# nullstyle/capnp-zig

Hardware: AMD Instinct MI355X
Metric: GiB/s device-resident packed encode+decode, 1M x 4KiB segments (higher is better)
Workload: dtype u8; 1 GPU; 1048576 units x 4096 B per GPU, zero-byte p=128/256, encode into capacity slots + decode from slots; units_per_gpu=1048576, unit_bytes=4096, zero_thresh=128, parallelism=shard1

## Files before the change

### capnp-zig_amd/csrc/packed_kernels.hip

```cpp
#include <hip/hip_runtime.h>
#include <stdint.h>
#include <stdio.h>
#include <stdlib.h>

#include <algorithm>
#include <atomic>
#include <map>
#include <memory>
#include <mutex>
#include <string>
#include <type_traits>
#include <vector>

#include "capnp_packed.h"
#include "class_ws.h"
#include "kernels.h"

namespace cpk {

constexpr int kWave = 64;
constexpr int kWavesPerBlock = 4;
constexpr int kBlock = kWave * kWavesPerBlock;

constexpr uint32_t kEncMaxWords = 512;
// ... 2808 lines not shown
                m_T = (uint32_t)(out_len[uu] >> 3);
                m_st = status[uu];
            }
        }
    };
    auto meta = [&](uint32_t j) {
        FillMeta m;
        m.st = (int32_t)readlane((uint32_t)m_st, j);
        m.P = readlane(m_P, j);
        m.src = in + ((uint64_t)readlane((uint32_t)m_in, j) | ((uint64_t)readlane((uint32_t)(m_in >> 32), j) << 32));
        m.dst = out + ((uint64_t)readlane((uint32_t)m_out, j) | ((uint64_t)readlane((uint32_t)(m_out >> 32), j) << 32));
        m.T = readlane(m_T, j);
        m.rec = reinterpret_cast<const uint16_t*>((uint64_t)readlane((uint32_t)m_rec, j) |
                                                  ((uint64_t)readlane((uint32_t)(m_rec >> 32), j) << 32));
        return m;
    };

    uint4 v0, v1, v2, v3, v4;
    uint32_t r0 = 0, r1 = 0, r2 = 0, r3 = 0, r4 = 0;
    auto load_unit = [&](const FillMeta& m) {
        const bool go = m.st == ST_OK && m.P > 0;
        if (!go) return;
        const uint32_t s = (uint32_t)(reinterpret_cast<uintptr_t>(m.src) & 15);
        const uint4* const b = reinterpret_cast<const uint4*>(m.src - s);
        const uint32_t np = (s + m.P + 15) >> 4;
        const uint32_t last = np - 1;
        v0 = load_nt(b + min(lane, last));
        if (np > 64) v1 = load_nt(b + min(lane + 64, last));
        if (np > 128) v2 = load_nt(b + min(lane + 128, last));
        if (np > 192) v3 = load_nt(b + min(lane + 192, last));
        if (np > 256) v4 = load_nt(b + min(lane + 256, last));
        const uint32_t L = (np + 63) >> 6;
        const uint16_t* const rc = m.rec;
        const uint32_t q = lane * L + 1;
        r0 = rc[min(q, np)];
        if (L > 1) r1 = rc[min(q + 1, np)];
        if (L > 2) r2 = rc[min(q + 2, np)];
        if (L > 3) r3 = rc[min(q + 3, np)];
        if (L > 4) r4 = rc[min(q + 4, np)];
    };

    load_batch(0);
    FillMeta cur = meta(0);
    load_unit(cur);
    uint32_t younger = 0;
    for (uint32_t k = 0; (uint64_t)u0 + (uint64_t)k * G < n; ++k) {
        const bool go = cur.st == ST_OK && cur.P > 0;
        vmcnt_at_most(younger);
        younger = 0;
        uint32_t np = 0, end = 0, pos = 0, words = 0, jend = 0;
        if (go) {
            const uint32_t s = (uint32_t)(reinterpret_cast<uintptr_t>(cur.src) & 15);
            end = s + cur.P;
            np = (end + 15) >> 4;
            wave_lds_sync();
            uint4* const pk4 = reinterpret_cast<uint4*>(pk);
            pk4[lane] = v0;
            if (np > 64) pk4[lane + 64] = v1;
            if (np > 128) pk4[lane + 128] = v2;
            if (np > 192) pk4[lane + 192] = v3;
            if (np > 256) pk4[lane + 256] = v4;
            const uint32_t L = (np + 63) >> 6;
            const uint32_t q0 = min(lane * L, np), q1 = min(q0 + L, np);
            const uint32_t nq = q1 - q0;
            jend = min(16 * q1, end);
            pos = jend;
            const uint32_t rr[kFlMaxL] = {r0, r1, r2, r3, r4};
#pragma unroll
            for (int i = kFlMaxL - 1; i >= 0; --i) {
                const uint32_t r = rr[i];
                const bool has = (uint32_t)i < nq && (r >> 4) != 0;
                words += has ? (r >> 4) : 0u;
                pos = has ? 16 * (q0 + i) + (r & 15u) : pos;
            }
        }
        const uint32_t k1 = k + 1;
        if ((k1 & 63) == 0) {
            asm volatile("s_waitcnt vmcnt(0)" ::: "memory");
            load_batch(k1);
        }
        const FillMeta nxt = meta(k1 & 63);
        load_unit(nxt);
        if (go) {
            const uint32_t incl = wave_incl_sum(words);
            const uint32_t wbase = incl - words;
            const bool a16 = !(reinterpret_cast<uintptr_t>(cur.dst) & 15);
            uint64_t* const dst = reinterpret_cast<uint64_t*>(cur.dst);
            const uint32_t T = cur.T;
            for (uint32_t W0 = 0; W0 < T; W0 += kFlOut) {
                const uint32_t W1 = min(T, W0 + kFlOut);
                wave_lds_sync();
                reinterpret_cast<uint4*>(code)[lane] = make_uint4(kFlZero * 0x10001u, kFlZero * 0x10001u,
                                                                  kFlZero * 0x10001u, kFlZero * 0x10001u);
                wave_lds_sync();
                const bool mine = words > 0 && wbase < W1 && wbase + words > W0;
                uint32_t p = mine ? pos : jend, w = wbase;
                bool runs = false;
                for (;;) {
                    const bool act = p < jend && w < W1;
                    if (__builtin_amdgcn_ballot_w64(act) == 0) break;
                    const uint32_t pp = act ? p : 0u;
                    uint32_t t = pk[pp];
                    uint32_t b1 = pk[pp + 1];
                    uint32_t c9 = pk[pp + 9];
                    asm volatile("" : "+v"(t), "+v"(b1), "+v"(c9));
                    const bool z = t == 0u, f = t == 0xFFu;
                    code[(act && !z && w >= W0) ? w - W0 : kFlOut] = (uint16_t)pp;
                    const uint32_t c = f ? c9 : 0u;
                    runs |= act && c != 0u;
                    if (act && c && w < W0) {
                        for (uint32_t i = W0 - w; i <= c && w + i < W1; ++i)
                            code[w + i - W0] = (uint16_t)(kFlLit | (pp + 1 + 8 * i));
                    }
                    w = act ? w + 1u + (z ? b1 : 0u) + c : w;
                    p = act ? p + 1u + __popc(t) + (uint32_t)(z | f) + 8u * c : p;
                }
                wave_lds_sync();
                if (__builtin_amdgcn_ballot_w64(runs) != 0) {
                    fl_bodies(pk, code, W1 - W0, lane);
                    wave_lds_sync();
                }
                const uint32_t nw = W1 - W0;
                if (a16) {
                    for (uint32_t i = 2 * lane; i < nw; i += 2 * kWave) {
                        const uint32_t cc = *reinterpret_cast<const uint32_t*>(code + i);
                        const uint64_t x0 = fill_word(pk, lut, cc & 0xFFFFu);
                        const uint64_t x1 = fill_word(pk, lut, cc >> 16);
                        if (i + 1 < nw) {
                            const u32x4 v = {(uint32_t)x0, (uint32_t)(x0 >> 32), (uint32_t)x1, (uint32_t)(x1 >> 32)};
                            __builtin_nontemporal_store(v, reinterpret_cast<u32x4*>(dst + W0 + i));
                        }
                        else dst[W0 + i] = x0;
                    }
                    younger += (nw + 2 * kWave - 1) / (2 * kWave);
                } else {
                    for (uint32_t i = lane; i < nw; i += kWave) dst[W0 + i] = fill_word(pk, lut, code[i]);
                    younger += (nw + kWave - 1) / kWave;
                }
            }
        }
        cur = nxt;
    }
    asm volatile("s_waitcnt vmcnt(0)" ::: "memory");
}

constexpr uint32_t kLwWaves = 2;
constexpr uint32_t kLwCarry = 12;
constexpr uint32_t kLwRing = kLwCarry + 64;
constexpr uint32_t kLwS = 8;
constexpr uint32_t kLwLine = 16;
constexpr uint32_t kLwLB = 8 * kLwLine;
constexpr uint32_t kLwLanes = kLwLB / 16;
constexpr uint32_t kLwLds = kLwWaves * kWave * (kLwRing + kLwLB + 2) + 128;
static_assert(kLwLds <= 26624, "six blocks per CU");

template <bool RD>
__global__ __launch_bounds__(kLwWaves * kWave) void decode_words_kernel(
    const uint8_t* __restrict__ in, const uint64_t* __restrict__ in_off, const uint64_t* __restrict__ in_len,
    uint32_t n, uint8_t* __restrict__ out, const uint64_t* __restrict__ out_off,
    const uint64_t* __restrict__ out_cap, uint64_t* __restrict__ out_len, int32_t* __restrict__ status,
    const uint32_t* __restrict__ list, const uint32_t* __restrict__ list_count,
    const uint32_t* __restrict__ list_lo, uint32_t* __restrict__ bail_count, uint64_t* __restrict__ consumed) {
    __shared__ __attribute__((aligned(16))) uint8_t ring_blk[kLwWaves * kWave * kLwRing];
    __shared__ __attribute__((aligned(16))) uint8_t line_blk[kLwWaves * kWave * kLwLB];
    __shared__ uint16_t ftab_blk[kLwWaves * kWave];
    __shared__ uint64_t nib[16];
    if (threadIdx.x < 16) {
        const uint64_t e = expand_selector(threadIdx.x);
        uint32_t m = 0;
        for (uint32_t k = 0; k < 4; ++k) m |= ((threadIdx.x >> k) & 1u) ? 0xFFu << (8 * k) : 0u;
        nib[threadIdx.x] = (e & 0xFFFFFFFFull) | ((uint64_t)m << 32);
    }
    __syncthreads();
    const uint32_t lane = lane_id();
    const uint32_t wave = threadIdx.x >> 6;
    uint8_t* const ring_all = ring_blk + wave * (kWave * kLwRing);
    uint8_t* const lines = line_blk + wave * (kWave * kLwLB);
    uint8_t* const myline = lines + lane * kLwLB;
    uint16_t* const ftab = ftab_blk + wave * kWave;
    const uint32_t wv = blockIdx.x * kLwWaves + wave;
    const uint32_t lo = list_lo ? *list_lo : 0u;
    const uint32_t count = (list ? *list_count : n) - lo;
    if (wv * kWave >= count) return;
    const uint32_t slot = wv * kWave + lane;
    const bool valid = slot < count;
    const uint32_t unit = valid ? ((list && (lo != 0 || count != n)) ? list[lo + slot] : slot) : 0u;

    const uint8_t* src = cpk_dummy16;
    uint64_t P64 = 0, cap = 0;
    uint8_t* dstb = nullptr;
    int32_t st = ST_OK;
    bool gated = false;
    uint64_t fw = 0;
    uint32_t past = 0;
    if (valid) {
        if (RD) gated = status[unit] != kStWords;
        src = in + in_off[unit];
        P64 = in_len[unit];
        dstb = out + out_off[unit];
        cap = out_cap[unit];
        if (RD) {
            fw = out_len[unit] >> 3;
            if (P64 > 10 * fw) {
                past = P64 - 10 * fw > (1u << 20) ? (1u << 20) : (uint32_t)(P64 - 10 * fw);
                P64 = 10 * fw;
            }
        }
        if (P64 > 0 && (reinterpret_cast<uintptr_t>(dstb) & 7)) st = ST_ARG;
        if (P64 >= kIxSizeMax) st = kStNeedFull;
    }
    const uint32_t s = (uint32_t)(reinterpret_cast<uintptr_t>(src) & 15);
    const bool take = valid && !gated && st == ST_OK && P64 > 0;
    const uint32_t end = take ? s + (uint32_t)P64 : 0u;
    const uint32_t npieces = (end + 15) >> 4;
    uint32_t maxr = (end + 63) >> 6;
#pragma unroll
    for (int d = 32; d >= 1; d >>= 1) maxr = max(maxr, (uint32_t)__shfl_xor((int)maxr, d, kWave));
    maxr = __builtin_amdgcn_readfirstlane(maxr);
    const uint32_t capw = (uint32_t)min(cap >> 3, (uint64_t)0x7FFFFFFFu);
    const uint32_t lim_w = RD ? (uint32_t)min(fw, (uint64_t)0x7FFFFFFFu) : capw;
    const uint32_t s0 = take ? (uint32_t)((reinterpret_cast<uintptr_t>(dstb) >> 3) & (kLwLine - 1)) : 0u;
    const uint64_t line0 = reinterpret_cast<uint64_t>(dstb) - 8ull * s0;

    const uint4* qsrc[4];
    uint32_t qlast[4];
#pragma unroll
    for (uint32_t m = 0; m < 4; ++m) {
        const uint32_t r = 16 * m + lane / 4;
        const uint64_t rb = __shfl(reinterpret_cast<uint64_t>(src - s), r, kWave);
        const uint32_t rn = __shfl(npieces, r, kWave);
        qsrc[m] = reinterpret_cast<const uint4*>(rn ? reinterpret_cast<const uint8_t*>(rb) : cpk_dummy16);
        qlast[m] = rn ? rn - 1 : 0u;
    }
    const uint32_t qp = lane & 3;
    u32x4 d0, d1, d2, d3;
    auto load = [&](uint32_t k) {
        ds_gload16(d0, qsrc[0] + min(4 * k + qp, qlast[0]));
        ds_gload16(d1, qsrc[1] + min(4 * k + qp, qlast[1]));
        ds_gload16(d2, qsrc[2] + min(4 * k + qp, qlast[2]));
        ds_gload16(d3, qsrc[3] + min(4 * k + qp, qlast[3]));
    };
    uint8_t* const wq = ring_all + (lane / 4) * kLwRing + kLwCarry + 16 * qp;
    auto put16 = [&](uint8_t* p, const u32x4& v) {
        uint32_t* const d = reinterpret_cast<uint32_t*>(p);
        d[0] = v.x;
        d[1] = v.y;
        d[2] = v.z;
        d[3] = v.w;
    };
    uint8_t* const ring = ring_all + lane * kLwRing;

    uint32_t younger = 0;
    auto flush = [&](bool want, uint64_t A, uint32_t lo, uint32_t hi) {
        const uint64_t F = __builtin_amdgcn_ballot_w64(want);
        if (F == 0) return;
        const uint32_t cnt = (uint32_t)__popcll(F);
        const uint32_t rk = __builtin_amdgcn_mbcnt_hi((uint32_t)(F >> 32), __builtin_amdgcn_mbcnt_lo((uint32_t)F, 0u));
        wave_lds_sync();
        if (want) ftab[rk] = (uint16_t)(lane | (lo << 6) | (hi << 10));
        wave_lds_sync();
        const uint32_t Alo = (uint32_t)A, Ahi = (uint32_t)(A >> 32);
        const uint32_t j = lane & (kLwLanes - 1);
        auto store16 = [&](uint32_t ent, uint64_t a, const u32x4& v, bool in_r) {
            const uint32_t flo = (ent >> 6) & 15u, fhi = ent >> 10;
            uint8_t* const p = reinterpret_cast<uint8_t*>(a) + 16 * j;
            if (__builtin_amdgcn_ballot_w64(in_r && (flo | (fhi ^ kLwLine)) != 0u) == 0) {
                ++younger;
                if (in_r) asm volatile("global_store_dwordx4 %0, %1, off nt\n\ts_nop 1" ::"v"(p), "v"(v));
                return;
            }
            const bool a0 = in_r && 2 * j >= flo && 2 * j < fhi, a1 = in_r && 2 * j + 1 >= flo && 2 * j + 1 < fhi;
            const bool both = a0 && a1, first = a0 && !a1, second = a1 && !a0;
            if (__builtin_amdgcn_ballot_w64(both) != 0) {
                ++younger;
                if (both) asm volatile("global_store_dwordx4 %0, %1, off nt\n\ts_nop 1" ::"v"(p), "v"(v));
            }
            if (__builtin_amdgcn_ballot_w64(first | second) != 0) {
                ++younger;
                uint8_t* const q = second ? p + 8 : p;
                const uint64_t x = second ? ((uint64_t)v.z | ((uint64_t)v.w << 32)) : ((uint64_t)v.x | ((uint64_t)v.y << 32));
                if (first | second) asm volatile("global_store_dwordx2 %0, %1, off nt\n\ts_nop 1" ::"v"(q), "v"(x));
            }
        };
        constexpr uint32_t kGrp = kWave / kLwLanes;
        for (uint32_t g = 0; g < cnt; g += 2 * kGrp) {
            const uint32_t ra = g + lane / kLwLanes, rb = ra + kGrp;
            const uint32_t ea = ftab[min(ra, cnt - 1)], eb = ftab[min(rb, cnt - 1)];
            const uint32_t ua = ea & 63u, ub = eb & 63u;
            const uint64_t aa = (uint64_t)(uint32_t)__shfl((int)Alo, (int)ua, kWave) |
                                ((uint64_t)(uint32_t)__shfl((int)Ahi, (int)ua, kWave) << 32);
            const uint64_t ab = (uint64_t)(uint32_t)__shfl((int)Alo, (int)ub, kWave) |
                                ((uint64_t)(uint32_t)__shfl((int)Ahi, (int)ub, kWave) << 32);
            const u32x4 va = *reinterpret_cast<const u32x4*>(lines + ua * kLwLB + 16 * j);
            const u32x4 vb = *reinterpret_cast<const u32x4*>(lines + ub * kLwLB + 16 * j);
            store16(ea, aa, va, ra < cnt);
            if (g + kGrp < cnt) store16(eb, ab, vb, rb < cnt);
        }
    };
    auto line_hi_cap = [&](uint32_t L, uint32_t hi) {
        const int64_t c = (int64_t)capw + s0 - (int64_t)kLwLine * L;
        return (uint32_t)max<int64_t>(0, min<int64_t>(hi, c));
    };

    constexpr int32_t kFar = 0x3FFFFFFF;
    int32_t po = take ? (int32_t)(s + kLwCarry) : kFar;
    int32_t end_o = take ? (int32_t)(end + kLwCarry) : 0;
    uint32_t run = 0, rsel = 0;
    int32_t apos = po;
    uint32_t W = 0;
    if (maxr > 0) load(0);
    uint32_t ksh = 0;
    for (uint32_t k = 0; k <= maxr; ++k) {
        if (__builtin_amdgcn_ballot_w64(take && W < lim_w && (po < end_o || run != 0u)) == 0) break;
        if (k < maxr) {
            vmcnt_at_most63(younger);
            asm volatile("" : "+v"(d0), "+v"(d1), "+v"(d2), "+v"(d3));
        }
        younger = 0;
        if (k > 0) {
            wave_lds_sync();
            uint32_t* const rd = reinterpret_cast<uint32_t*>(ring);
            const uint32_t c0 = rd[16], c1 = rd[17], c2 = rd[18];
            rd[0] = c0;
            rd[1] = c1;
            rd[2] = c2;
            wave_lds_sync();
            po -= 64;
            end_o -= 64;
            ++ksh;
            apos = apos == INT32_MIN ? apos : po;
        }
        if (k < maxr) {
            put16(wq, d0);
            put16(wq + 16 * kLwRing, d1);
            put16(wq + 32 * kLwRing, d2);
            put16(wq + 48 * kLwRing, d3);
            if (k + 1 < maxr) load(k + 1);
            wave_lds_sync();
        }
        const int32_t lim = min(64, end_o);
        const int32_t slim = min(67, end_o);
        for (;;) {
            if (__builtin_amdgcn_ballot_w64(run >= kLwLine && rsel == 0u) != 0) {
                const uint32_t wcap = min(lim_w, capw);
                const bool bz = rsel == 0u && run >= kLwLine && ((s0 + W) & (kLwLine - 1)) == 0u &&
                                W + kLwLine <= wcap;
                if (__builtin_amdgcn_ballot_w64(bz) != 0) {
                    const uint32_t nl = bz ? min(run, wcap - W) / kLwLine : 0u;
                    const uint32_t nmax = wave_max_u32(nl);
                    const u32x4 z = {0u, 0u, 0u, 0u};
                    for (uint32_t i = 0; i < nmax; ++i) {
                        if (i < nl) {
                            uint8_t* const zl = reinterpret_cast<uint8_t*>(line0 + (uint64_t)kLwLB * ((s0 + W) / kLwLine + i));
#pragma unroll
                            for (uint32_t c = 0; c < kLwLB / 16; ++c)
                                asm volatile("global_store_dwordx4 %0, %1, off nt\n\ts_nop 1" ::"v"(zl + 16 * c), "v"(z));
                        }
                        younger += kLwLB / 16;
                    }
                    W += kLwLine * nl;
                    run -= kLwLine * nl;
                    apos = (run != 0u && rsel == 0u) ? INT32_MIN : po;
                }
            }
            uint32_t rec[kLwS];
#pragma unroll
            for (uint32_t j = 0; j < kLwS; ++j) rec[j] = 0u;
            uint32_t e = 0;
            __builtin_amdgcn_s_setprio(1);
            const uint32_t rem = W < lim_w ? lim_w - W : 0u;
            const int32_t limx = rem != 0u ? slim : INT32_MIN;
#pragma unroll
            for (uint32_t j = 0; j < kLwS; ++j) {
                const bool act = apos < limx && (!RD || j < rem);
                if (__builtin_amdgcn_ballot_w64(act) == 0) break;
                if (act) {
                    const uint32_t o = (uint32_t)min(max(po, 0), 66);
                    const uint8_t* const a = ring + o;
                    uint32_t t = a[0], b1 = a[1], c9 = a[9];
                    asm volatile("" : "+v"(t), "+v"(b1), "+v"(c9));
                    const bool inrec = run == 0u;
                    const bool tz = t == 0u, tf = t == 0xFFu;
                    const uint32_t len = (uint32_t)__popc(t) + 1u + (uint32_t)(tz | tf);
                    const uint32_t cnt = tz ? b1 : (tf ? c9 : 0u);
                    const uint32_t tsel = inrec ? t : rsel;
                    rec[j] = (o + (uint32_t)inrec) | (tsel << 8);
                    po += (int32_t)(inrec ? len : (rsel & 8u));
                    run = inrec ? cnt : run - 1u;
                    rsel = inrec ? (tf ? 0xFFu : 0u) : rsel;
                    apos = (run != 0u && rsel == 0u) ? INT32_MIN : po;
                    e = j + 1;
                }
            }
            __builtin_amdgcn_s_setprio(0);
            uint64_t w[kLwS];
#pragma unroll
            for (uint32_t j = 0; j < kLwS; ++j) {
                const uint32_t r16 = rec[j];
                const uint32_t o = r16 & 0xFFu, sh = o & 3u;
                const uint32_t* const rw = reinterpret_cast<const uint32_t*>(ring + (o & ~3u));
                const uint32_t D0 = rw[0], D1 = rw[1], D2 = rw[2];
                const uint64_t pay = (uint64_t)__builtin_amdgcn_alignbyte(D1, D0, sh) |
                                     ((uint64_t)__builtin_amdgcn_alignbyte(D2, D1, sh) << 32);
                const uint32_t tg = r16 >> 8;
                const uint64_t elo = nib[tg & 15u], ehi = nib[tg >> 4];
                const uint32_t shi = (uint32_t)ehi + (((uint32_t)__popc(tg & 15u) * 0x01010101u) & (uint32_t)(ehi >> 32));
                w[j] = perm64(pay, (uint64_t)(uint32_t)elo | ((uint64_t)shi << 32));
            }
            const uint32_t sl = (s0 + W) & (kLwLine - 1);
            const uint32_t f = kLwLine - sl;
#pragma unroll
            for (uint32_t j = 0; j < kLwS; ++j)
                if (j < e && j < f) *reinterpret_cast<uint64_t*>(myline + 8 * ((sl + j) & (kLwLine - 1))) = w[j];
            const bool full = e >= f && e != 0u;
            if (__builtin_amdgcn_ballot_w64(full) != 0) {
                __builtin_amdgcn_s_setprio(1);
                const uint32_t L = (s0 + W) / kLwLine;
                flush(full, line0 + (uint64_t)kLwLB * L, L == 0 ? s0 : 0u, line_hi_cap(L, kLwLine));
                __builtin_amdgcn_s_setprio(0);
                wave_lds_sync();
#pragma unroll
                for (uint32_t j = 0; j < kLwS; ++j)
                    if (j < e && j >= f) *reinterpret_cast<uint64_t*>(myline + 8 * ((sl + j) & (kLwLine - 1))) = w[j];
            }
            W += e;
            if (__builtin_amdgcn_ballot_w64(apos < lim && W < lim_w) == 0) break;
        }
    }
    {
        const uint32_t L = (s0 + W) / kLwLine, hi = (s0 + W) & (kLwLine - 1);
        const bool part = take && hi != 0u;
        flush(part, line0 + (uint64_t)kLwLB * L, L == 0 ? s0 : 0u, line_hi_cap(L, hi));
    }
    asm volatile("s_waitcnt vmcnt(0)" ::: "memory");
    if (!valid || gated) return;
    if (st == kStNeedFull) {
        status[unit] = st;
        return;
    }
    if (RD) {
        const int32_t rend = po + (int32_t)((rsel & 8u) * run);
        int32_t rs = st;
        if (rs == ST_OK && take)
            rs = (W < lim_w || po > end_o) ? ST_EOS
                                           : (run != 0u ? (rend > end_o + (int32_t)past ? ST_EOS : ST_OVERSHOOT) : ST_OK);
        if (rs != ST_OK) {
            out_len[unit] = 0;
            consumed[unit] = 0;
            status[unit] = rs;
            return;
        }
        consumed[unit] = take ? (uint64_t)((int64_t)po + 64ll * ksh - kLwCarry - s) : 0ull;
        out_len[unit] = 8ull * W;
        status[unit] = 8ull * W > cap ? ST_SPACE : ST_OK;
        return;
    }
    if (take && (po != end_o || run != 0u)) {
        if (W >= lim_w && po <= end_o) {
            status[unit] = kStNeedFull;
            atomicAdd(bail_count, 1u);
            return;
        }
        st = ST_EOF;
    }
    if (st != ST_OK) {
        out_len[unit] = 0;
        status[unit] = st;
        return;
    }
    out_len[unit] = 8ull * W;
    status[unit] = 8ull * W > cap ? ST_SPACE : ST_OK;
}


enum : uint32_t { CL_LONG = 0, CL_HUGE = 1, CL_SMALL = 2, CL_MID = 3 };
constexpr uint32_t kEsBinsQ = 4;
constexpr uint64_t kSmEncWords = 64;
constexpr uint64_t kSmDecP = 512;
constexpr uint64_t kSmDecCap = 8192;
constexpr uint64_t kMidSplitP = 1280;
constexpr uint64_t kWordsCapMax = 8192;

__device__ __forceinline__ uint32_t* q_blocks(uint32_t* q, uint32_t n) { return q + block_counts_off(n); }

template <int KIND>
__device__ __forceinline__ uint32_t unit_class(const uint8_t* in, const uint64_t* in_off, const uint64_t* in_len,
                                               uint8_t* out, const uint64_t* out_off, const uint64_t* out_cap,
                                               uint32_t u) {
    const uint64_t off = in_off[u], len = in_len[u];
    if (KIND == 2) {
        const uint64_t s = reinterpret_cast<uintptr_t>(in + off) & 15;
        if (len > 0 && ((s + len + 15) >> 4) > kFlPieces) return len > kQHuge ? CL_HUGE : CL_LONG;
        return CL_MID;
    }
    if (KIND == 4) {
        if (encode_tiled_unit(in, off, len)) return len > kQHuge ? CL_HUGE : CL_LONG;
        const bool valid = !(reinterpret_cast<uintptr_t>(in + off) & 7) && !(len & 7);
        const bool small = !valid || (len >> 3) <= kSmEncWords;
        const uint64_t w = len >> 3;
        return !small ? CL_MID : CL_MID + 4 + (valid && w > 8) + (valid && w > 16) + (valid && w > 32);
    }
    const uint64_t cap = out_cap[u];
    if (len <= kSmDecP && cap <= kSmDecCap) return CL_SMALL;
    if (decode_long_unit(in, off, len, out, out_off[u], cap)) return len > kQHuge ? CL_HUGE : CL_LONG;
    if (cap > kWordsCapMax) return CL_MID + (len > 768) + (len > 1024);
    return CL_MID + (len > 768) + (len > 1024) + (len > kMidSplitP) + (len > 1536) + (len > 2048) + (len > 2560) +
           (len > 3072);
}

template <int KIND>
__global__ __launch_bounds__(kClassBlock) void class_count_kernel(const uint8_t* __restrict__ in,
                                                                  const uint64_t* __restrict__ in_off,
                                                                  const uint64_t* __restrict__ in_len, uint32_t n,
                                                                  uint8_t* __restrict__ out,
                                                                  const uint64_t* __restrict__ out_off,
                                                                  const uint64_t* __restrict__ out_cap, uint32_t* q,
                                                                  int32_t* __restrict__ status) {
    __shared__ uint32_t cnt[kClassK];
    if (threadIdx.x < kClassK) cnt[threadIdx.x] = 0;
    __syncthreads();
    const uint32_t u = blockIdx.x * kClassBlock + threadIdx.x;
    const uint32_t c = u < n ? unit_class<KIND>(in, in_off, in_len, out, out_off, out_cap, u) : kClassK;
    if (c <= CL_HUGE) status[u] = kStPending;
#pragma unroll
    for (uint32_t k = 0; k < kClassK; ++k) {
        const uint64_t m = __ballot(c == k);
        if (m && lane_id() == 0) atomicAdd(&cnt[k], (uint32_t)__popcll(m));
    }
    __syncthreads();
    if (threadIdx.x < kClassK) q_blocks(q, n)[blockIdx.x * kClassK + threadIdx.x] = cnt[threadIdx.x];
}

__global__ __launch_bounds__(1024) void class_scan_kernel(uint32_t* q, uint32_t n, uint32_t nb, uint32_t words_min) {
    __shared__ uint32_t wsum[16][kClassK];
    __shared__ uint32_t carry[kClassK];
    uint32_t* const bl = q_blocks(q, n);
    const uint32_t lane = lane_id(), w = threadIdx.x >> 6;
    if (threadIdx.x < kClassK) carry[threadIdx.x] = 0;
    if (threadIdx.x < kQHead) q[threadIdx.x] = 0u;
    __syncthreads();
    for (uint32_t b0 = 0; b0 < nb; b0 += 1024) {
        const uint32_t b = b0 + threadIdx.x;
        uint32_t v[kClassK], incl[kClassK];
#pragma unroll
        for (uint32_t k = 0; k < kClassK; ++k) {
            v[k] = b < nb ? bl[b * kClassK + k] : 0u;
            incl[k] = wave_incl_sum(v[k]);
            if (lane == 63) wsum[w][k] = incl[k];
        }
        __syncthreads();
#pragma unroll
        for (uint32_t k = 0; k < kClassK; ++k) {
            uint32_t pre = carry[k];
            for (uint32_t j = 0; j < w; ++j) pre += wsum[j][k];
            if (b < nb) bl[b * kClassK + k] = pre + incl[k] - v[k];
        }
        __syncthreads();
        if (threadIdx.x < kClassK) {
            uint32_t t = 0;
            for (uint32_t j = 0; j < 16; ++j) t += wsum[j][threadIdx.x];
            carry[threadIdx.x] += t;
        }
        __syncthreads();
    }
    if (threadIdx.x == 0) {
        q[kSlotLong] = carry[CL_LONG];
        q[kSlotHuge] = carry[CL_HUGE];
        q[kSlotSmall] = carry[CL_SMALL];
        uint32_t mid = 0;
        for (uint32_t b = 0; b < CL_MID_BINS; ++b) {
            q[kSlotMidBefore + b] = mid;
            mid += carry[CL_MID + b];
        }
        q[kSlotMid] = mid;
        const uint32_t over = mid - q[kSlotMidBefore + 3];
        q[kSlotTwoPass] = words_min == 0 ? 0u : (over >= words_min ? q[kSlotMidBefore + 3] : mid);
        q[kSlotCapped] = 0;
    }
}

template <int KIND>
__global__ __launch_bounds__(kClassBlock) void class_scatter_kernel(const uint8_t* __restrict__ in,
                                                                    const uint64_t* __restrict__ in_off,
                                                                    const uint64_t* __restrict__ in_len, uint32_t n,
                                                                    uint8_t* __restrict__ out,
                                                                    const uint64_t* __restrict__ out_off,
                                                                    const uint64_t* __restrict__ out_cap, uint32_t* q,
                                                                    uint32_t fused, uint32_t words_min) {
    __shared__ uint32_t wcnt[16][kClassK];
    __shared__ uint32_t wtot[16][kClassK];
    __shared__ uint32_t pre_s[kClassK], own_s[kClassK], tot_s[kClassK], midb_s[CL_MID_BINS + 1];
    const uint32_t lane = lane_id(), w = threadIdx.x >> 6;
    const uint32_t u = blockIdx.x * kClassBlock + threadIdx.x;
    const uint32_t nb = gridDim.x;
    uint32_t v[kClassK];
    if (fused) {
        const uint32_t* const bl = q_blocks(q, n);
#pragma unroll
        for (uint32_t k = 0; k < kClassK; ++k) v[k] = threadIdx.x < nb ? bl[threadIdx.x * kClassK + k] : 0u;
    }
    const uint32_t c = u < n ? unit_class<KIND>(in, in_off, in_len, out, out_off, out_cap, u) : kClassK;
    if (fused) {
#pragma unroll
        for (uint32_t k = 0; k < kClassK; ++k) {
            const uint32_t a = wave_incl_sum(v[k]);
            if (lane == 63) wtot[w][k] = a;
            if (threadIdx.x == blockIdx.x) {
                own_s[k] = v[k];
                pre_s[k] = a - v[k];
            }
        }
    }
    uint32_t rank = 0;
#pragma unroll
    for (uint32_t k = 0; k < kClassK; ++k) {
        const uint64_t m = __ballot(c == k);
        if (lane == 0) wcnt[w][k] = (uint32_t)__popcll(m);
        if (c == k) rank = (uint32_t)__popcll(m & ((1ull << lane) - 1ull));
    }
    __syncthreads();
    if (fused) {
        if (threadIdx.x < kClassK) {
            const uint32_t wb = blockIdx.x >> 6;
            uint32_t a = 0, b = 0;
            for (uint32_t j = 0; j < 16; ++j) {
                a += wtot[j][threadIdx.x];
                b += j < wb ? wtot[j][threadIdx.x] : 0u;
            }
            tot_s[threadIdx.x] = a;
            pre_s[threadIdx.x] += b;
        }
        __syncthreads();
        if (threadIdx.x == 0) {
            uint32_t mid = 0;
            for (uint32_t b = 0; b < CL_MID_BINS; ++b) {
                midb_s[b] = mid;
                mid += tot_s[CL_MID + b];
            }
            midb_s[CL_MID_BINS] = mid;
        }
        __syncthreads();
        if (blockIdx.x == 0 && threadIdx.x < kQHead) {
            const uint32_t t = threadIdx.x, mid = midb_s[CL_MID_BINS];
            uint32_t v = 0;
            if (t == kSlotLong) v = tot_s[CL_LONG];
            else if (t == kSlotHuge) v = tot_s[CL_HUGE];
            else if (t == kSlotSmall) v = tot_s[CL_SMALL];
            else if (t == kSlotMid) v = mid;
            else if (t >= kSlotMidBefore && t < kSlotMidBefore + CL_MID_BINS) v = midb_s[t - kSlotMidBefore];
            else if (t == kSlotTwoPass) v = words_min == 0 ? 0u : (mid - midb_s[3] >= words_min ? midb_s[3] : mid);
            q[t] = v;
        }
    }
    if (c >= kClassK) return;
    const uint32_t* const P = q_blocks(q, n);
    const uint32_t pc = fused ? pre_s[c] : P[blockIdx.x * kClassK + c];
    uint32_t idx = pc + rank;
    for (uint32_t j = 0; j < w; ++j) idx += wcnt[j][c];
    if (KIND == 4 && c >= CL_MID + CL_MID_BINS - kEsBinsQ) {
        uint32_t before = 0;
        for (uint32_t cc = CL_MID + CL_MID_BINS - kEsBinsQ; cc < CL_MID + CL_MID_BINS; ++cc) {
            const uint32_t b = cc - CL_MID;
            uint32_t pb, pn;
            if (fused) {
                pb = pre_s[cc];
                pn = pb + own_s[cc];
            } else {
                const uint32_t tot = q[mid_through_slot(b)] - q[kSlotMidBefore + b];
                pb = P[blockIdx.x * kClassK + cc];
                pn = blockIdx.x + 1 < nb ? P[(blockIdx.x + 1) * kClassK + cc] : tot;
            }
            before += pb + (cc < c ? pn - pb : 0u);
        }
        idx = before + (idx - pc);
        const uint32_t base = fused ? midb_s[CL_MID_BINS - kEsBinsQ] : q[kSlotMidBefore + CL_MID_BINS - kEsBinsQ];
        q[mid_list_off(n) + base + idx] = u;
        return;
    }
    if (c == CL_LONG) q[long_slot(idx)] = u;
    else if (c == CL_HUGE) q[huge_slot(n, idx)] = u;
    else if (c == CL_SMALL) q[small_list_off(n) + idx] = u;
    else q[mid_list_off(n) + (fused ? midb_s[c - CL_MID] : q[kSlotMidBefore + (c - CL_MID)]) + idx] = u;
}

constexpr uint32_t kTileSkip = 0xFFFFFFFFu;
struct TileTab {
    uint64_t* size;
    uint32_t* unit;
    uint32_t* first;
    uint32_t* serial;
    uint64_t cap;
};
static_assert(sizeof(*TileTab::size) + sizeof(*TileTab::unit) + sizeof(*TileTab::first) == kTileEntBytes,
              "tile table entry");
__device__ __forceinline__ TileTab tile_tab(uint32_t* q, uint32_t n) {
    TileTab t;
    t.cap = tile_cap(n);
    t.serial = q + serial_off(n);
    t.size = reinterpret_cast<uint64_t*>(q + tile_tab_off(n));
    t.unit = q + tile_tab_off(n) + tile_unit_col(t.cap);
    t.first = t.unit + t.cap;
    return t;
}
__device__ __forceinline__ unsigned long long* q_tiles(uint32_t* q) {
    return reinterpret_cast<unsigned long long*>(q + kSlotReserved);
}

__device__ __forceinline__ uint64_t wave_reserve(unsigned long long* ctr, uint64_t k) {
    const uint32_t lane = lane_id();
    uint64_t incl = k;
#pragma unroll
    for (int d = 1; d < kWave; d <<= 1) {
        const uint64_t o = __shfl_up(incl, d, kWave);
        if (lane >= (uint32_t)d) incl += o;
    }
    const uint64_t total = __shfl(incl, kWave - 1, kWave);
    uint64_t b = 0;
    if (lane == 0 && total != 0) b = atomicAdd(ctr, (unsigned long long)total);
    b = __shfl(b, 0, kWave);
    return b + incl - k;
}

__global__ __launch_bounds__(256) void long_tiles_kernel(const uint64_t* __restrict__ in_len, uint32_t n, uint32_t* q) {
    const uint32_t nh = q[kSlotHuge], nl = q[kSlotLong];
    const TileTab t = tile_tab(q, n);
    for (uint32_t i0 = blockIdx.x * 256 + (threadIdx.x & ~(kWave - 1)); i0 < nl + nh; i0 += gridDim.x * 256) {
    const uint32_t i = i0 + lane_id();
    const bool v = i < nl + nh;
    const uint32_t unit = !v ? 0u : q[long_list_slot(n, nh, i)];
    const uint64_t k = v ? ((in_len[unit] >> 3) + kEncMaxWords - 1) / kEncMaxWords : 0ull;
// ... 2366 lines not shown
```

Baseline: 1284 GiB/s.

## Software-pipeline packed decode: expand previous step's words during current tag scan

Restructures the wave-level packed decode loop so that payload extraction happens during the tag scan. Expansion, LDS line writes and flushing of the previous iteration's words are deferred and interleaved with the current iteration's serial tag parsing. Payloads and tags are carried across iterations in registers, with a drain step after the loop. The intent is to hide the latency of the serial tag-walk dependency chain under independent expansion work. In exchange it uses more VGPRs, always executes all kLwS slots because the early ballot break is gone, and adds a retire delay that could affect correctness at edges.

```diff
diff --git a/capnp-zig_amd/csrc/packed_kernels.hip b/capnp-zig_amd/csrc/packed_kernels.hip
--- a/capnp-zig_amd/csrc/packed_kernels.hip
+++ b/capnp-zig_amd/csrc/packed_kernels.hip
@@ -3134,6 +3134,31 @@
         return (uint32_t)max<int64_t>(0, min<int64_t>(hi, c));
     };
 
+    uint64_t pw[kLwS], xw[kLwS];
+#pragma unroll
+    for (uint32_t j = 0; j < kLwS; ++j) pw[j] = 0, xw[j] = 0;
+    uint32_t ptl = 0, pth = 0, pe = 0, pW = 0;
+    auto ptag = [&](uint32_t j) { return ((j < 4 ? ptl : pth) >> (8 * (j & 3))) & 0xFFu; };
+    auto nib_lo = [&](uint32_t n) { return reinterpret_cast<const uint32_t*>(nib)[2 * n]; };
+    auto expand = [&](uint64_t pay, uint32_t tlo, uint32_t elo, uint64_t ehi) {
+        const uint32_t shi = (uint32_t)ehi + (((uint32_t)__popc(tlo) * 0x01010101u) & (uint32_t)(ehi >> 32));
+        return perm64(pay, (uint64_t)elo | ((uint64_t)shi << 32));
+    };
+    auto retire = [&]() {
+        const uint32_t sl = (s0 + pW) & (kLwLine - 1), f = kLwLine - sl;
+        const bool full = pe >= f && pe != 0u;
+        if (__builtin_amdgcn_ballot_w64(full) != 0) {
+            __builtin_amdgcn_s_setprio(1);
+            const uint32_t L = (s0 + pW) / kLwLine;
+            flush(full, line0 + (uint64_t)kLwLB * L, L == 0 ? s0 : 0u, line_hi_cap(L, kLwLine));
+            __builtin_amdgcn_s_setprio(0);
+            wave_lds_sync();
+#pragma unroll
+            for (uint32_t j = 0; j < kLwS; ++j)
+                if (j < pe && j >= f) *reinterpret_cast<uint64_t*>(myline + 8 * ((sl + j) & (kLwLine - 1))) = xw[j];
+        }
+    };
+
     constexpr int32_t kFar = 0x3FFFFFFF;
     int32_t po = take ? (int32_t)(s + kLwCarry) : kFar;
     int32_t end_o = take ? (int32_t)(end + kLwCarry) : 0;
@@ -3195,69 +3220,62 @@
                     apos = (run != 0u && rsel == 0u) ? INT32_MIN : po;
                 }
             }
-            uint32_t rec[kLwS];
-#pragma unroll
-            for (uint32_t j = 0; j < kLwS; ++j) rec[j] = 0u;
-            uint32_t e = 0;
+            uint32_t ctl = 0u, cth = 0u, e = 0;
+            const uint32_t psl = (s0 + pW) & (kLwLine - 1);
+            const uint32_t pf = kLwLine - psl;
             __builtin_amdgcn_s_setprio(1);
             const uint32_t rem = W < lim_w ? lim_w - W : 0u;
             const int32_t limx = rem != 0u ? slim : INT32_MIN;
+            uint32_t elo = nib_lo(ptag(0) & 15u);
+            uint64_t ehi = nib[ptag(0) >> 4];
 #pragma unroll
             for (uint32_t j = 0; j < kLwS; ++j) {
                 const bool act = apos < limx && (!RD || j < rem);
-                if (__builtin_amdgcn_ballot_w64(act) == 0) break;
+                const uint32_t o = (uint32_t)min(max(po, 0), 66);
+                const bool inrec = run == 0u;
+                const uint32_t op = o + (uint32_t)inrec;
+                const uint8_t* const a = ring + o;
+                uint32_t t = a[0], b1 = a[1], c9 = a[9];
+                const uint32_t* const rw = reinterpret_cast<const uint32_t*>(ring + (op & ~3u));
+                const uint32_t D0 = rw[0], D1 = rw[1], D2 = rw[2];
+                uint32_t nlo = 0;
+                uint64_t nhi = 0;
+                if (j + 1 < kLwS) nlo = nib_lo(ptag(j + 1) & 15u), nhi = nib[ptag(j + 1) >> 4];
+                xw[j] = expand(pw[j], ptag(j) & 15u, elo, ehi);
+                if (j < pe && j < pf) *reinterpret_cast<uint64_t*>(myline + 8 * ((psl + j) & (kLwLine - 1))) = xw[j];
+                elo = nlo, ehi = nhi;
                 if (act) {
-                    const uint32_t o = (uint32_t)min(max(po, 0), 66);
-                    const uint8_t* const a = ring + o;
-                    uint32_t t = a[0], b1 = a[1], c9 = a[9];
                     asm volatile("" : "+v"(t), "+v"(b1), "+v"(c9));
-                    const bool inrec = run == 0u;
                     const bool tz = t == 0u, tf = t == 0xFFu;
                     const uint32_t len = (uint32_t)__popc(t) + 1u + (uint32_t)(tz | tf);
                     const uint32_t cnt = tz ? b1 : (tf ? c9 : 0u);
                     const uint32_t tsel = inrec ? t : rsel;
-                    rec[j] = (o + (uint32_t)inrec) | (tsel << 8);
+                    (j < 4 ? ctl : cth) |= tsel << (8 * (j & 3));
                     po += (int32_t)(inrec ? len : (rsel & 8u));
                     run = inrec ? cnt : run - 1u;
                     rsel = inrec ? (tf ? 0xFFu : 0u) : rsel;
                     apos = (run != 0u && rsel == 0u) ? INT32_MIN : po;
                     e = j + 1;
+                    const uint32_t sh = op & 3u;
+                    pw[j] = (uint64_t)__builtin_amdgcn_alignbyte(D1, D0, sh) |
+                            ((uint64_t)__builtin_amdgcn_alignbyte(D2, D1, sh) << 32);
                 }
             }
             __builtin_amdgcn_s_setprio(0);
-            uint64_t w[kLwS];
-#pragma unroll
-            for (uint32_t j = 0; j < kLwS; ++j) {
-                const uint32_t r16 = rec[j];
-                const uint32_t o = r16 & 0xFFu, sh = o & 3u;
-                const uint32_t* const rw = reinterpret_cast<const uint32_t*>(ring + (o & ~3u));
-                const uint32_t D0 = rw[0], D1 = rw[1], D2 = rw[2];
-                const uint64_t pay = (uint64_t)__builtin_amdgcn_alignbyte(D1, D0, sh) |
-                                     ((uint64_t)__builtin_amdgcn_alignbyte(D2, D1, sh) << 32);
-                const uint32_t tg = r16 >> 8;
-                const uint64_t elo = nib[tg & 15u], ehi = nib[tg >> 4];
-                const uint32_t shi = (uint32_t)ehi + (((uint32_t)__popc(tg & 15u) * 0x01010101u) & (uint32_t)(ehi >> 32));
-                w[j] = perm64(pay, (uint64_t)(uint32_t)elo | ((uint64_t)shi << 32));
-            }
-            const uint32_t sl = (s0 + W) & (kLwLine - 1);
-            const uint32_t f = kLwLine - sl;
-#pragma unroll
-            for (uint32_t j = 0; j < kLwS; ++j)
-                if (j < e && j < f) *reinterpret_cast<uint64_t*>(myline + 8 * ((sl + j) & (kLwLine - 1))) = w[j];
-            const bool full = e >= f && e != 0u;
-            if (__builtin_amdgcn_ballot_w64(full) != 0) {
-                __builtin_amdgcn_s_setprio(1);
-                const uint32_t L = (s0 + W) / kLwLine;
-                flush(full, line0 + (uint64_t)kLwLB * L, L == 0 ? s0 : 0u, line_hi_cap(L, kLwLine));
-                __builtin_amdgcn_s_setprio(0);
-                wave_lds_sync();
-#pragma unroll
-                for (uint32_t j = 0; j < kLwS; ++j)
-                    if (j < e && j >= f) *reinterpret_cast<uint64_t*>(myline + 8 * ((sl + j) & (kLwLine - 1))) = w[j];
-            }
+            retire();
+            ptl = ctl, pth = cth, pe = e, pW = W;
             W += e;
             if (__builtin_amdgcn_ballot_w64(apos < lim && W < lim_w) == 0) break;
         }
+    }
+    if (__builtin_amdgcn_ballot_w64(pe != 0u) != 0) {
+        const uint32_t psl = (s0 + pW) & (kLwLine - 1), pf = kLwLine - psl;
+#pragma unroll
+        for (uint32_t j = 0; j < kLwS; ++j) {
+            xw[j] = expand(pw[j], ptag(j) & 15u, nib_lo(ptag(j) & 15u), nib[ptag(j) >> 4]);
+            if (j < pe && j < pf) *reinterpret_cast<uint64_t*>(myline + 8 * ((psl + j) & (kLwLine - 1))) = xw[j];
+        }
+        retire();
     }
     {
         const uint32_t L = (s0 + W) / kLwLine, hi = (s0 + W) & (kLwLine - 1);
```

After: 1294 GiB/s, median of 6. No clear change (+0.8%).
